# jonH34400/3DBodyAnimation

Measured on AMD Instinct MI355X. Metric: SMPL residual+Jacobian evals/sec (6890v, 10 beta, 24 joints), higher is better.
Workload: dtype f64 residual/Jacobian; f32 mesh (f32 + split-bf16 MFMA blend); 1 GPU; C3: 256 independent frames per GPU, BODY_25 (14 FK joints + 11 vertex landmarks), opt-shape (per-frame beta, 86 cols), GMM prior on, 6890-vertex mesh on; frames_per_gpu=256, keypoints_per_frame=25, n_cols=86

## Files before the change

### 3dbodyanimation_amd/csrc/frame_part_inl.h

```cpp
#pragma once
#include <hip/hip_ext.h>

#include "bodyfit_device.h"
#include "priors_inl.h"

namespace bodyfit {
namespace {

__device__ __forceinline__ void store_through(double* p, double v) {
  __hip_atomic_store(p, v, __ATOMIC_RELAXED, __HIP_MEMORY_SCOPE_SYSTEM);
}
#ifndef BODYFIT_J_THROUGH
#define BODYFIT_J_THROUGH 1
#endif
template <bool kFused>
__device__ __forceinline__ void store_J(double* p, double v, int scope = 0) {
  if constexpr (kFused && !BODYFIT_J_THROUGH) *p = v;
  else if (scope == 1) store_f64_through(p, v);
  else if (scope == 2) *p = v;
  else store_through(p, v);
}


__device__ inline void mul33(const double* A, const double* B, double* C) {
#pragma unroll
  for (int r = 0; r < 3; ++r)
#pragma unroll
    for (int c = 0; c < 3; ++c) C[r * 3 + c] = A[r * 3] * B[c] + A[r * 3 + 1] * B[3 + c] + A[r * 3 + 2] * B[6 + c];
}
__device__ inline void mul33_bt(const double* A, const double* B, double* C) {
#pragma unroll
  for (int r = 0; r < 3; ++r)
#pragma unroll
    for (int c = 0; c < 3; ++c)
      C[r * 3 + c] = A[r * 3] * B[c * 3] + A[r * 3 + 1] * B[c * 3 + 1] + A[r * 3 + 2] * B[c * 3 + 2];
}
__device__ inline void mv3(const double* A, double x0, double x1, double x2, double* y) {
#pragma unroll
  for (int r = 0; r < 3; ++r) y[r] = A[r * 3] * x0 + A[r * 3 + 1] * x1 + A[r * 3 + 2] * x2;
}

__device__ void rodrigues_grad_k(double a0, double a1, double a2, int k, double* R, double* dRk) {
  const double th2 = a0 * a0 + a1 * a1 + a2 * a2;
  if (th2 > 2.220446049250313e-16) {
    const double th = sqrt(th2), ith = 1.0 / th;
    double sh, ch;
    sincos(0.5 * th, &sh, &ch);
    const double st = 2.0 * sh * ch, omc = 2.0 * sh * sh, ct = 1.0 - omc;
    const double w[3] = {a0 * ith, a1 * ith, a2 * ith};
    const double K[9] = {0, -w[2], w[1], w[2], 0, -w[0], -w[1], w[0], 0};
#pragma unroll
    for (int r = 0; r < 3; ++r)
#pragma unroll
      for (int c = 0; c < 3; ++c) R[r * 3 + c] = (r == c ? ct : 0.0) + st * K[r * 3 + c] + omc * w[r] * w[c];
    const double wk = (k == 0) ? w[0] : (k == 1 ? w[1] : w[2]);
    double dw[3];
#pragma unroll
    for (int i = 0; i < 3; ++i) dw[i] = ((i == k ? 1.0 : 0.0) - w[i] * wk) * ith;
    const double dK[9] = {0, -dw[2], dw[1], dw[2], 0, -dw[0], -dw[1], dw[0], 0};
#pragma unroll
    for (int r = 0; r < 3; ++r)
#pragma unroll
      for (int c = 0; c < 3; ++c)
        dRk[r * 3 + c] = (r == c ? -st * wk : 0.0) + ct * wk * K[r * 3 + c] + st * dK[r * 3 + c] +
                         st * wk * w[r] * w[c] + omc * (dw[r] * w[c] + w[r] * dw[c]);
  } else {
    R[0] = 1; R[1] = -a2; R[2] = a1;
    R[3] = a2; R[4] = 1; R[5] = -a0;
    R[6] = -a1; R[7] = a0; R[8] = 1;
#pragma unroll
    for (int i = 0; i < 9; ++i) dRk[i] = 0.0;
    if (k == 0) { dRk[5] = -1; dRk[7] = 1; }
    else if (k == 1) { dRk[2] = 1; dRk[6] = -1; }
    else { dRk[1] = -1; dRk[3] = 1; }
  }
}

__device__ inline double wave_sum(double v) {
#pragma unroll
  for (int off = 32; off > 0; off >>= 1) v += __shfl_down(v, off, 64);
  return v;
}

#ifdef BODYFIT_STAMPS
#define STAMP(i)                                                                              \
  do {                                                                                        \
    if (Pb.dbg && (threadIdx.x & 63) == 0) {                                                  \
      unsigned long long t_;                                                                  \
      asm volatile("s_memtime %0\n\ts_waitcnt lgkmcnt(0)" : "=s"(t_)::"memory");              \
      Pb.dbg[((size_t)f * 8 + (threadIdx.x >> 6)) * 16 + (i)] = t_;                  \
    }                                                                                         \
  } while (0)
#define STAMP_REAL(i)                                                                         \
  do {                                                                                        \
    if (Pb.dbg && (threadIdx.x & 63) == 0) {                                                  \
      unsigned long long t_;                                                                  \
      asm volatile("s_memrealtime %0\n\ts_waitcnt lgkmcnt(0)" : "=s"(t_)::"memory");          \
      Pb.dbg[((size_t)f * 8 + (threadIdx.x >> 6)) * 16 + (i)] = t_;                  \
    }                                                                                         \
  } while (0)
#else
#define STAMP(i)
#define STAMP_REAL(i)
#endif

constexpr int KC = 32;
constexpr int kThreads = 512;

constexpr int OFF_X = 0;
constexpr int OFF_R = OFF_X + 88;
constexpr int OFF_DR = OFF_R + 216;
constexpr int OFF_A = OFF_DR + 648;
constexpr int OFF_P = OFF_A + 216;
constexpr int OFF_O = OFF_P + 72;
constexpr int OFF_JC = OFF_O + 72;
constexpr int OFF_W = OFF_JC + 72;
constexpr int OFF_B = OFF_W + 624;
constexpr int OFF_FEAT = OFF_B + 720;
constexpr int OFF_CAM = OFF_FEAT + 208;
constexpr int OFF_KP = OFF_CAM + 40;
constexpr int OFF_TAB = OFF_KP + KC * 18;
constexpr int OFF_KPUV = OFF_TAB + 64;
constexpr int OFF_DS = OFF_KPUV + 2 * KC;
constexpr int OFF_SC = OFF_DS + 720;
constexpr int OFF_PART = OFF_SC + 720;
constexpr int OFF_T = OFF_PART + 128;
constexpr int OFF_CHAIN = OFF_T + 720;
constexpr int OFF_LM = OFF_CHAIN + 24;
constexpr int LM_VP = 0;
constexpr int LM_Q = 3;
constexpr int LM_A = 6;
constexpr int LM_X = 15;
constexpr int LM_W = 39;
constexpr int LM_J = 47;
constexpr int LM_NW = 51;
constexpr int LM_BETA = 52;
constexpr int LM_PD = 82;
constexpr int LM_STRIDE = 290;
constexpr int TAB_PARENT = 0;
constexpr int TAB_ANC = 24;
constexpr int TAB_KPID = 96;

struct FrameHead {
  const unsigned char* mtab;
  const unsigned char* ptab;
  const double* R0;
  int F, K;
  int dims;
};
static_assert(kMaxJoints < 64 && kMaxShape < 16 && kMaxLandmarks < 64 && 7 + 3 * (kMaxJoints - 1) + kMaxShape < 256,
              "FrameHead::dims: 6 + 4 + 6 + 8 bits for nJ, nS, nL, ncols; beta_stride (0 or nS) in 4");
__host__ __device__ inline int frame_head_dims(int nJ, int nS, int nL, int ncols, int use_shape, int beta_stride, int has_coef) {
  return nJ | (nS << 6) | (nL << 10) | (ncols << 16) | ((use_shape ? 1 : 0) << 24) | (beta_stride << 25) | ((has_coef ? 1 : 0) << 29);
}

struct FusedFrame {
  unsigned* flag;
  unsigned epoch;
  int j_scope;
};

template <bool kFused>
__device__ __forceinline__ void frame_sync() {
  if constexpr (kFused) asm volatile("s_waitcnt lgkmcnt(0)\n\ts_barrier" ::: "memory");
  else __syncthreads();
}

template <bool kFused>
__device__ __forceinline__ void store_operand16(void* p, uint4 v) {
  if constexpr (kFused) {
    typedef __attribute__((ext_vector_type(4))) unsigned int u32x4_;
    const u32x4_ x = {v.x, v.y, v.z, v.w};
    asm volatile("global_store_dwordx4 %0, %1, off sc1\n\ts_nop 1" ::"v"(p), "v"(x) : "memory");
  } else {
    *reinterpret_cast<uint4*>(p) = v;
  }
}

template <bool kFused>
__device__ __forceinline__ void frame_part(const DevModel& M, const DevProblem& Pb, const double* __restrict__ params,
                                           const double* __restrict__ beta, double* __restrict__ r_out,
                                           double* __restrict__ J_out, double* __restrict__ joints_out, const MeshCoef& mc,
                                           int want_jac, double* sm, int f, const FusedFrame& fu, const FrameHead& hd) {
  const int tid = threadIdx.x;
  const int lane = tid & 63, wave = tid >> 6;
  const int nJ = kFused ? (hd.dims & 63) : M.nJ, nS = kFused ? ((hd.dims >> 6) & 15) : M.nS, nL = kFused ? ((hd.dims >> 10) & 63) : M.nL;
  const int ncols = kFused ? ((hd.dims >> 16) & 255) : Pb.ncols;
  const int npose = 7 + 3 * (nJ - 1);
  const bool use_shape = kFused ? (((hd.dims >> 24) & 1) != 0) : (Pb.use_shape != 0);
  const int beta_stride = kFused ? ((hd.dims >> 25) & 15) : Pb.beta_stride;
  const unsigned char* const mtab = kFused ? hd.mtab : M.tabA;
  const unsigned char* const ptab = kFused ? hd.ptab : Pb.ptab;
  const int* const t_parent = reinterpret_cast<const int*>(mtab + kTabParent);
  const unsigned* const t_anc = reinterpret_cast<const unsigned*>(mtab + kTabAnc);
  const unsigned long long* const t_chain = reinterpret_cast<const unsigned long long*>(mtab + kTabChain);
  const int* const t_lm_woff = reinterpret_cast<const int*>(mtab + kTabLmWoff);
  const int* const t_lm_wj = reinterpret_cast<const int*>(mtab + kTabLmWj);
  const double* const t_lm_ww = reinterpret_cast<const double*>(mtab + kTabLmWw);
  const double* const t_lm_vt = reinterpret_cast<const double*>(mtab + kTabLmVt);
  const double* const t_lm_sd = reinterpret_cast<const double*>(mtab + kTabLmSd);
  const double* const t_dS = reinterpret_cast<const double*>(mtab + kTabDS);
  const double* const t_Sc = reinterpret_cast<const double*>(mtab + kTabSc);
  const double* const t_offset = reinterpret_cast<const double*>(mtab + kTabOffset);
  const double* const t_Jc0 = reinterpret_cast<const double*>(mtab + kTabJc0);
  const int t_F = kFused ? hd.F : Pb.F, t_K = kFused ? hd.K : Pb.K;
  const int* const t_kp_offset = reinterpret_cast<const int*>(ptab);
  const int* const t_kp_id = reinterpret_cast<const int*>(ptab + ptab_id_off(t_F));
  const double* const t_kp_uv = reinterpret_cast<const double*>(ptab + ptab_uv_off(t_F, t_K));
  const double* const t_R0 = kFused ? hd.R0 : Pb.R0;
  const int P = M.P;
  double* sx = sm + OFF_X;
  double* sR = sm + OFF_R;
  double* sdR = sm + OFF_DR;
  double* sA = sm + OFF_A;
  double* sP = sm + OFF_P;
  double* sO = sm + OFF_O;
  double* sJc = sm + OFF_JC;
  double* sW = sm + OFF_W;
  double* sB = sm + OFF_B;
  double* sFeat = sm + OFF_FEAT;
  double* sCam = sm + OFF_CAM;
  double* sKp = sm + OFF_KP;
  int* sTab = reinterpret_cast<int*>(sm + OFF_TAB);
  double* sKpUv = sm + OFF_KPUV;
  double* sDS = sm + OFF_DS;
  double* sSc = sm + OFF_SC;
  double* sPart = sm + OFF_PART;
  double* sLm = sm + OFF_LM;
  double* sT = sm + OFF_T;
  double* sLmSd = sLm + nL * LM_STRIDE;
  int* sParent = sTab + TAB_PARENT;
  unsigned* sAnc = reinterpret_cast<unsigned*>(sTab + TAB_ANC);
  int* sKpId = sTab + TAB_KPID;
  unsigned* sKpAnc = reinterpret_cast<unsigned*>(sTab + 48);
  unsigned long long* sChain = reinterpret_cast<unsigned long long*>(sm + OFF_CHAIN);

  STAMP_REAL(10);
  STAMP(0);
#ifdef BODYFIT_STAMPS
  if (Pb.dbg && tid == 0) {
    unsigned xcc;
    asm volatile("s_getreg_b32 %0, hwreg(HW_REG_XCC_ID)" : "=s"(xcc));
    Pb.dbg[((size_t)f * 8) * 16 + 9] = xcc & 0xf;
  }
#endif
  if constexpr (!kFused) {
    if (Pb.frame_flags && !(Pb.frame_flags[f] & Pb.frame_mask)) return;
  }
  constexpr int kLoaders = kThreads;
  constexpr bool loader = true;
  constexpr int kSdPasses = (kMaxLandmarks * 3 * kMaxShape + kThreads - 1) / kThreads;
  constexpr int kPasses = (720 + kLoaders - 1) / kLoaders;
  const bool coef_wave = kFused && wave == 5 && ((hd.dims >> 29) & 1) != 0;
  const int tj_c = min(tid, nJ - 1);
  const int par_in = t_parent[tj_c];
  const unsigned anc_in = t_anc[tj_c];
  const unsigned long long chain_in = t_chain[tj_c];
  const int nlw = nL * kMaxLmNnz, lw_i = min(tid, max(nlw, 1) - 1);
  const double lww_in = t_lm_ww[lw_i];
  const int lwj_in = t_lm_wj[lw_i];
  const int lwo_in = t_lm_woff[lw_i / kMaxLmNnz];
  const int nsd = nL * 3 * nS, nds = nJ * 3 * nS;
  double sd_in[kSdPasses], t0[kPasses], t1[kPasses];
#pragma unroll
  for (int u = 0; u < kSdPasses; ++u) sd_in[u] = t_lm_sd[min(tid + u * kThreads, max(nsd, 1) - 1)];
#pragma unroll
  for (int u = 0; u < kPasses; ++u) {
    const int i = min(tid + u * kLoaders, max(nds, 1) - 1);
    t0[u] = t_dS[i];
    t1[u] = t_Sc[i];
  }
  const int k_begin0 = t_kp_offset[f], nk0 = min(KC, t_kp_offset[f + 1] - k_begin0);
  const int o_i = tid - 128, v_row = tid - 256;
  const bool o_lane = tid >= 128 && o_i < nJ * 3, v_lane = tid >= 256 && v_row < nL * 3;
  double o_pre = 0.0, jc_pre = 0.0, vt_pre = 0.0;
  if (o_lane) { o_pre = t_offset[o_i]; jc_pre = t_Jc0[o_i]; }
  if (v_lane) vt_pre = t_lm_vt[v_row];
  const int cam_lane = tid - 384;
  const bool cam_on = cam_lane >= 0 && cam_lane < 36;
  double r0c0 = 0.0, r0c1 = 0.0, r0c2 = 0.0;
  if (cam_on) {
    const double* R0 = t_R0 + (size_t)f * 9;
    const int c = cam_lane % 3;
    r0c0 = R0[c]; r0c1 = R0[3 + c]; r0c2 = R0[6 + c];
  }
  double x_in = 0.0;
  const bool x_lane = tid >= 128 && tid - 128 < npose, b_lane = tid >= 224 && tid - 224 < nS;
  if (x_lane) x_in = params[(size_t)f * npose + tid - 128];
  if (b_lane) x_in = (use_shape && beta) ? beta[(size_t)f * beta_stride + tid - 224] : 0.0;
  int kp_id0 = 0;
  double kp_u0 = 0.0, kp_v0 = 0.0;
  if (loader) {
    kp_id0 = t_kp_id[k_begin0 + (tid & (KC - 1))];
    kp_u0 = t_kp_uv[2 * (size_t)(k_begin0 + (tid & (KC - 1)))];
    kp_v0 = t_kp_uv[2 * (size_t)(k_begin0 + (tid & (KC - 1))) + 1];
  }
  if (tid < nJ) { sParent[tid] = par_in; sAnc[tid] = anc_in; sChain[tid] = chain_in; }
  volatile int* sWalkDone = reinterpret_cast<volatile int*>(sPart + 104);
  if (tid == 0) *sWalkDone = 0;
  if (tid < nlw) {
    const int l = tid / kMaxLmNnz, i = tid % kMaxLmNnz;
    double* L = sLm + l * LM_STRIDE;
    L[LM_W + i] = lww_in;
    reinterpret_cast<int*>(L + LM_J)[i] = lwj_in;
    if (i == 0) L[LM_NW] = (double)lwo_in;
  }
#pragma unroll
  for (int u = 0; u < kSdPasses; ++u)
    if (tid + u * kThreads < nsd) sLmSd[tid + u * kThreads] = sd_in[u];
#pragma unroll
  for (int u = 0; u < kPasses; ++u) {
    const int i = tid + u * kLoaders;
    if (i < nds) { sDS[i] = t0[u]; sSc[i] = t1[u]; }
  }
  if (x_lane) sx[tid - 128] = x_in;
  if (b_lane) sx[npose + tid - 224] = x_in;
  frame_sync<kFused>();
  if (tid < nk0) {
    sTab[TAB_KPID + tid] = kp_id0;
    sKpUv[2 * tid] = kp_u0;
    sKpUv[2 * tid + 1] = kp_v0;
  }
  const double* sbeta = sx + npose;

  STAMP(1);
  if (tid < 3 * nJ) {
    const int jj = tid / 3, k = tid - 3 * jj;
    const double* aa = (jj == 0) ? (sx + 1) : (sx + 7 + 3 * (jj - 1));
    double R[9], dRk[9];
    rodrigues_grad_k(aa[0], aa[1], aa[2], k, R, dRk);
    if (k == 0) {
#pragma unroll
      for (int i = 0; i < 9; ++i) sR[jj * 9 + i] = R[i];
    }
#pragma unroll
    for (int i = 0; i < 9; ++i) sdR[jj * 27 + k * 9 + i] = dRk[i];
  }
  if (v_lane) {
    const int row = v_row;
    double sv[kMaxShape];
#pragma unroll
    for (int k = 0; k < kMaxShape; ++k) sv[k] = (use_shape && k < nS) ? sLmSd[row * nS + k] : 0.0;
    double acc = vt_pre;
#pragma unroll
    for (int k = 0; k < kMaxShape; ++k) acc += sv[k] * sbeta[min(k, nS > 0 ? nS - 1 : 0)];
    sPart[row] = acc;
  }
  if (coef_wave) {
    float* cf = reinterpret_cast<float*>(sW);
    const int nfeat = 9 * (nJ - 1);
    if (lane < nJ - 1) {
      const float a0 = (float)sx[7 + 3 * lane], a1 = (float)sx[8 + 3 * lane], a2 = (float)sx[9 + 3 * lane];
      const float th2 = a0 * a0 + a1 * a1 + a2 * a2;
      float st = 1.0f, omc = 0.0f, w0 = a0, w1 = a1, w2 = a2;
      if (th2 > 1e-20f) {
        const float ith = rsqrtf(th2), th = th2 * ith;
        float sh, ch;
        sincosf(0.5f * th, &sh, &ch);
        st = 2.0f * sh * ch; omc = 2.0f * sh * sh;
        w0 = a0 * ith; w1 = a1 * ith; w2 = a2 * ith;
      }
      const float on = Pb.pose_blend ? 1.0f : 0.0f;
      float* o = cf + 9 * lane;
      o[0] = on * (omc * (w0 * w0 - 1.0f)); o[1] = on * (omc * w0 * w1 - st * w2); o[2] = on * (omc * w0 * w2 + st * w1);
      o[3] = on * (omc * w1 * w0 + st * w2); o[4] = on * (omc * (w1 * w1 - 1.0f)); o[5] = on * (omc * w1 * w2 - st * w0);
      o[6] = on * (omc * w2 * w0 - st * w1); o[7] = on * (omc * w2 * w1 + st * w0); o[8] = on * (omc * (w2 * w2 - 1.0f));
    } else if (lane >= 32 && lane - 32 < 16 * kBlendKSteps - kPoseFeat) {
      const int i = lane - 32;
      cf[kPoseFeat + i] = (i < nS) ? (float)sbeta[i] : ((i == kMaxShape || i == kMaxShape + 1) ? 1.0f : 0.0f);
    }
    if (lane < 32)
      for (int k = nfeat + lane; k < kPoseFeat; k += 32) cf[k] = 0.0f;
  }
  if (o_lane) {
    const int i = o_i;
    double o = o_pre, jc = jc_pre;
    if (use_shape) {
      for (int k = 0; k < nS; ++k) {
        o += sDS[i * nS + k] * sbeta[k];
        jc += sSc[i * nS + k] * sbeta[k];
      }
    }
    sO[i] = (i < 3) ? 0.0 : o;
    if (i < 3) sPart[100 + i] = o;
    sJc[i] = jc;
  }
  __builtin_amdgcn_s_waitcnt(0x0F70);
  frame_sync<kFused>();

  STAMP(2);
  const int lm_k = lane & 31, lm_l = 2 * wave + (lane >> 5);
  const bool lm_blend = Pb.pose_blend && P > 0;
  auto lm_load = [&](int l, double (&pdv)[27]) {
    const double* row = M.lm_pd + (size_t)min(l, max(nL, 1) - 1) * 27 * 32 + lm_k;
#pragma unroll
    for (int ae = 0; ae < 27; ++ae) pdv[ae] = row[ae * 32];
  };
  auto lm_terms = [&](int l, const double (&pdv)[27]) {
    const int k = min(lm_k + 1, nJ - 1);
    const bool lm_on = l < nL, on = lm_on && lm_k < nJ - 1;
    const double onf = (lm_blend && on) ? 1.0 : 0.0;
    double part[3] = {0.0, 0.0, 0.0};
#pragma unroll
    for (int e = 0; e < 9; ++e) {
      const double fe = (sR[k * 9 + e] - ((e % 4 == 0) ? 1.0 : 0.0)) * onf;
#pragma unroll
      for (int a = 0; a < 3; ++a) part[a] += pdv[a * 9 + e] * fe;
    }
    if (want_jac) {
#pragma unroll
      for (int c = 0; c < 3; ++c) {
        const double* d = sdR + k * 27 + c * 9;
        double h[3] = {0.0, 0.0, 0.0};
#pragma unroll
        for (int e = 0; e < 9; ++e) {
          const double de = d[e] * onf;
#pragma unroll
          for (int a = 0; a < 3; ++a) h[a] += pdv[a * 9 + e] * de;
        }
        if (on) {
          double* o = sLm + l * LM_STRIDE + LM_PD + (3 * (k - 1) + c) * 3;
          o[0] = h[0]; o[1] = h[1]; o[2] = h[2];
        }
      }
    }
#pragma unroll
    for (int a = 0; a < 3; ++a) {
#pragma unroll
      for (int off = 16; off > 0; off >>= 1) part[a] += __shfl_xor(part[a], off, 32);
    }
    if (lm_on && lm_k == 0) {
#pragma unroll
      for (int a = 0; a < 3; ++a) sLm[l * LM_STRIDE + LM_VP + a] = sPart[l * 3 + a] + part[a];
    }
  };
  const bool lm_wave0 = 2 * wave < nL, lm_wave1 = 2 * wave + 16 < nL;
  if (tid < 9) sA[tid] = (tid % 4 == 0) ? 1.0 : 0.0;
  if (tid >= 16 && tid < 19) sP[tid - 16] = 0.0;
  if (tid >= 32 && tid - 32 < 3 * nS) { sB[tid - 32] = 0.0; sT[tid - 32] = 0.0; }
  if (wave == 0) {
    asm volatile("s_waitcnt lgkmcnt(0)" ::: "memory");
    if (lane == 0) __hip_atomic_fetch_add(const_cast<int*>(sWalkDone), 1, __ATOMIC_RELAXED, __HIP_MEMORY_SCOPE_WORKGROUP);
  }
  if (coef_wave) {
    const float* cf = reinterpret_cast<const float*>(sW);
    if (lane < kBlendKSteps * 4) {
      const int kstep = lane >> 2, h = (lane >> 1) & 1, hl = lane & 1;
      const float4 v0 = *reinterpret_cast<const float4*>(cf + 16 * kstep + 8 * h);
      const float4 v1 = *reinterpret_cast<const float4*>(cf + 16 * kstep + 8 * h + 4);
      const float x[8] = {v0.x, v0.y, v0.z, v0.w, v1.x, v1.y, v1.z, v1.w};
      uint32_t pk[4];
#pragma unroll
      for (int q = 0; q < 4; ++q) {
        uint16_t b[2];
#pragma unroll
        for (int t = 0; t < 2; ++t) {
          const uint16_t hi = f32_to_bf16(x[2 * q + t]);
          b[t] = hl == 0 ? hi : f32_to_bf16(x[2 * q + t] - bf16_to_f32(hi));
        }
        pk[q] = (uint32_t)b[0] | ((uint32_t)b[1] << 16);
      }
      const int ftile = f / kFTile, phi = f % kFTile;
      const int row = 8 * (phi >> 3) + 4 * (phi & 1) + ((phi >> 1) & 3);
      uint4* dst = reinterpret_cast<uint4*>(reinterpret_cast<unsigned char*>(mc.featA) + ((size_t)ftile * kBlendKSteps + kstep) * 2048 +
                                            feat_frag_off(h * 32 + row, hl));
      store_operand16<true>(dst, make_uint4(pk[0], pk[1], pk[2], pk[3]));
    }
    asm volatile("s_waitcnt vmcnt(0)" ::: "memory");
    STAMP_REAL(14);
    if (lane == 0)
      (void)__hip_atomic_fetch_add(fu.flag + (size_t)(f / kFTile) * kUnitCounterStride + kUnitCoefOffset, 1u, __ATOMIC_RELAXED,
                                   __HIP_MEMORY_SCOPE_AGENT);
  }
  double pdv0[27];
  if (lm_wave0) lm_load(lm_l, pdv0);
  for (int i = tid; i < 208; i += kThreads) {
    double v = 0.0;
    if (i < 9 * (nJ - 1)) v = sR[9 + i] - (((i % 9) % 4 == 0) ? 1.0 : 0.0);
    sFeat[i] = v;
  }
  auto walk = [&](int kind, int j, int sel, bool on) {
    j = on ? j : 1;
    const double* tab = (kind == 2) ? sDS : sO;
    const int stride = (kind == 2) ? nS : 1, off = (kind == 2) ? sel : 0;
    const double m = (kind == 0) ? 0.0 : 1.0;
    const double* ini = (kind == 0) ? (sR + j * 9 + sel) : (tab + (j * 3) * stride + off);
    const int istride = (kind == 0) ? 3 : stride;
    double v0 = ini[0], v1 = ini[istride], v2 = ini[2 * istride];
    unsigned long long ch = on ? sChain[j] : 0ull;
    int k = (int)(ch & 31ull);
    double Rc[9], oc[3];
    auto fetch = [&](int kk, double (&Rn)[9], double (&on_)[3]) {
#pragma unroll
      for (int e = 0; e < 9; ++e) Rn[e] = sR[kk * 9 + e];
#pragma unroll
      for (int a3 = 0; a3 < 3; ++a3) on_[a3] = tab[(kk * 3 + a3) * stride + off];
    };
    fetch(k, Rc, oc);
    while (k > 0) {
      ch >>= 5;
      const int kn = (int)(ch & 31ull);
      double Rn[9], on_[3];
      fetch(kn, Rn, on_);
      const double t0 = Rc[0] * v0 + Rc[1] * v1 + Rc[2] * v2 + m * oc[0];
      const double t1 = Rc[3] * v0 + Rc[4] * v1 + Rc[5] * v2 + m * oc[1];
      const double t2 = Rc[6] * v0 + Rc[7] * v1 + Rc[8] * v2 + m * oc[2];
      v0 = t0; v1 = t1; v2 = t2;
#pragma unroll
      for (int e = 0; e < 9; ++e) Rc[e] = Rn[e];
      oc[0] = on_[0]; oc[1] = on_[1]; oc[2] = on_[2];
      k = kn;
    }
    if (!on) return;
    if (kind == 0) { sA[j * 9 + sel] = v0; sA[j * 9 + 3 + sel] = v1; sA[j * 9 + 6 + sel] = v2; }
    else if (kind == 1) { sP[j * 3] = v0; sP[j * 3 + 1] = v1; sP[j * 3 + 2] = v2; }
    else {
      sB[(j * 3 + 0) * nS + sel] = v0; sB[(j * 3 + 1) * nS + sel] = v1; sB[(j * 3 + 2) * nS + sel] = v2;
      double c[3];
      mv3(sA + j * 9, sSc[(j * 3 + 0) * nS + sel], sSc[(j * 3 + 1) * nS + sel], sSc[(j * 3 + 2) * nS + sel], c);
      sT[(j * 3 + 0) * nS + sel] = v0 - c[0]; sT[(j * 3 + 1) * nS + sel] = v1 - c[1]; sT[(j * 3 + 2) * nS + sel] = v2 - c[2];
    }
  };
  if (!kFused && wave == 0 && mc.featA) {
    const int ftile = f / kFTile, phi = f % kFTile;
    const int row = Pb.feat_perm ? (8 * (phi >> 3) + 4 * (phi & 1) + ((phi >> 1) & 3)) : phi;
    if (lane >= 8 && lane - 8 < kBlendKSteps * 4) {
      const int wl = lane - 8;
      const int kstep = wl >> 2, h = (wl >> 1) & 1, hl = wl & 1;
      const int k0 = kstep * 16 + 8 * h;
      const int nfeat = 9 * (nJ - 1);
      double vr[8], vb[8];
#pragma unroll
      for (int u = 0; u < 8; ++u) {
        vr[u] = sR[9 + min(k0 + u, nfeat - 1)];
        vb[u] = sbeta[min(max(k0 + u - kPoseFeat, 0), max(nS, 1) - 1)];
      }
      uint32_t pk[4];
#pragma unroll
      for (int jj = 0; jj < 4; ++jj) {
        uint16_t b[2];
#pragma unroll
        for (int u = 0; u < 2; ++u) {
          const int k = k0 + 2 * jj + u;
          const float xr = (Pb.pose_blend && k < nfeat) ? (float)(vr[2 * jj + u] - (((k % 9) % 4 == 0) ? 1.0 : 0.0)) : 0.0f;
          const float xb = (k - kPoseFeat < nS) ? (float)vb[2 * jj + u]
                                                : ((k == kPoseFeat + kMaxShape || k == kPoseFeat + kMaxShape + 1) ? 1.0f : 0.0f);
          const float x = (k < kPoseFeat) ? xr : xb;
          const uint16_t hi = f32_to_bf16(x);
          b[u] = hl == 0 ? hi : f32_to_bf16(x - bf16_to_f32(hi));
        }
        pk[jj] = (uint32_t)b[0] | ((uint32_t)b[1] << 16);
      }
      uint4* dst = reinterpret_cast<uint4*>(reinterpret_cast<unsigned char*>(mc.featA) + ((size_t)ftile * kBlendKSteps + kstep) * 2048 +
                                            feat_frag_off(h * 32 + row, hl));
      store_operand16<kFused>(dst, make_uint4(pk[0], pk[1], pk[2], pk[3]));
    }
  }
  if (cam_on) {
    const int mtx = cam_lane / 9, e = cam_lane % 9, r = e / 3;
    const double* Lm = (mtx == 0) ? sR : (sdR + (mtx - 1) * 9);
    sCam[cam_lane] = Lm[r * 3] * r0c0 + Lm[r * 3 + 1] * r0c1 + Lm[r * 3 + 2] * r0c2;
  }
  {
    const int nA = 3 * (nJ - 1), nP = nJ - 1;
    const int nA6 = (nA + 1) / 2, nP6 = (nP + 1) / 2;
    if (wave == 6 || wave == 7) {
      const int a0 = wave == 6 ? 0 : nA6, na = wave == 6 ? nA6 : nA - nA6;
      const int p0 = wave == 6 ? 0 : nP6, np = wave == 6 ? nP6 : nP - nP6;
      const bool isA = lane < na, isP = !isA && lane - na < np;
      const int item = isA ? a0 + lane : p0 + (lane - na);
      walk(isA ? 0 : 1, isA ? 1 + item / 3 : 1 + item, isA ? item % 3 : 0, isA || isP);
    }
  }
  if (wave == 6) {
    asm volatile("s_waitcnt lgkmcnt(0)" ::: "memory");
    if (lane == 0) __hip_atomic_fetch_add(const_cast<int*>(sWalkDone), 256, __ATOMIC_RELAXED, __HIP_MEMORY_SCOPE_WORKGROUP);
  }
  if (wave == 7) {
    STAMP(13);
    for (int spin = 0; spin < (1 << 20) && *sWalkDone < 257; ++spin) __builtin_amdgcn_s_sleep(1);
    asm volatile("" ::: "memory");
    STAMP(14);
    const double s_ = sx[0];
    const double* Rr0_ = sCam;
    for (int it = lane; it < 3 * nJ; it += 64) {
      const int jj = it / 3, r = it - 3 * jj;
      const double* Aj = sA + jj * 9;
      const double a0 = Rr0_[r * 3], a1 = Rr0_[r * 3 + 1], a2 = Rr0_[r * 3 + 2];
      double q[3];
      mv3(Aj, sJc[jj * 3], sJc[jj * 3 + 1], sJc[jj * 3 + 2], q);
      const double p0 = sP[jj * 3], p1 = sP[jj * 3 + 1], p2 = sP[jj * 3 + 2];
      if (mc.skinT) {
        const double ra0 = a0 * Aj[0] + a1 * Aj[3] + a2 * Aj[6];
        const double ra1 = a0 * Aj[1] + a1 * Aj[4] + a2 * Aj[7];
        const double ra2 = a0 * Aj[2] + a1 * Aj[5] + a2 * Aj[8];
        const double tr = a0 * (p0 - q[0]) + a1 * (p1 - q[1]) + a2 * (p2 - q[2]);
        float4* T = reinterpret_cast<float4*>(mc.skinT + (size_t)f * nJ * 12) + it;
        store_operand16<kFused>(T, make_uint4(__float_as_uint((float)(s_ * ra0)), __float_as_uint((float)(s_ * ra1)),
                                              __float_as_uint((float)(s_ * ra2)), __float_as_uint((float)(s_ * tr + sx[4 + r]))));
      }
      if (joints_out) joints_out[(size_t)f * nJ * 3 + it] = s_ * (a0 * p0 + a1 * p1 + a2 * p2) + sx[4 + r];
    }
    STAMP(15);
    if constexpr (kFused) {
      asm volatile("s_waitcnt vmcnt(0)" ::: "memory");
      STAMP_REAL(9);
      if (lane == 0)
        (void)__hip_atomic_fetch_add(fu.flag + (size_t)(f / kFTile) * kUnitCounterStride, 1u, __ATOMIC_RELAXED, __HIP_MEMORY_SCOPE_AGENT);
      STAMP_REAL(12);
    }
  }
  if (lm_wave0) lm_terms(lm_l, pdv0);
  if (lm_wave1) {
    double pdv1[27];
    lm_load(lm_l + 16, pdv1);
    lm_terms(lm_l + 16, pdv1);
  }
  STAMP(3);
  frame_sync<kFused>();

  STAMP(4);
  if (use_shape && want_jac) {
    for (int it = tid - 192; it >= 0 && tid < 448 && it < nS * (nJ - 1); it += 256) walk(2, 1 + it / nS, it % nS, true);
  }
  if (want_jac && tid < 3 * (nJ - 1)) {
    const int k = 1 + tid / 3, c = tid % 3, p = sParent[k];
    double T1[9], T2[9], Wm[9];
    mul33_bt(sdR + k * 27 + c * 9, sR + k * 9, T1);
    mul33(sA + p * 9, T1, T2);
    mul33_bt(T2, sA + p * 9, Wm);
#pragma unroll
    for (int e = 0; e < 9; ++e) sW[tid * 9 + e] = Wm[e];
  }
  if (wave == 2 && lane < nL) {
    double* L = sLm + lane * LM_STRIDE;
    const int* Lj = reinterpret_cast<const int*>(L + LM_J);
    double q[3] = {0, 0, 0}, Ab[9] = {0, 0, 0, 0, 0, 0, 0, 0, 0};
    const int nw = (int)L[LM_NW];
    for (int i = 0; i < nw; ++i) {
      const int j = Lj[i];
      const double w = L[LM_W + i];
      double xj[3];
      mv3(sA + j * 9, L[LM_VP] - sJc[j * 3], L[LM_VP + 1] - sJc[j * 3 + 1], L[LM_VP + 2] - sJc[j * 3 + 2], xj);
#pragma unroll
      for (int a = 0; a < 3; ++a) {
        xj[a] += sP[j * 3 + a];
        q[a] += w * xj[a];
        L[LM_X + i * 3 + a] = xj[a];
      }
#pragma unroll
      for (int e = 0; e < 9; ++e) Ab[e] += w * sA[j * 9 + e];
    }
#pragma unroll
    for (int a = 0; a < 3; ++a) L[LM_Q + a] = q[a];
#pragma unroll
    for (int e = 0; e < 9; ++e) L[LM_A + e] = Ab[e];
  }
  if (wave == 2 && M.lm_gcount) {
    const int cnt = (lane < nL) ? M.lm_gcount[lane] : 0;
    if (cnt > 1) {
      double* L = sLm + lane * LM_STRIDE;
      double q0 = L[LM_Q], q1 = L[LM_Q + 1], q2 = L[LM_Q + 2];
      for (int i = 1; i < cnt; ++i) {
        const double* Li = L + i * LM_STRIDE;
        q0 += Li[LM_Q]; q1 += Li[LM_Q + 1]; q2 += Li[LM_Q + 2];
      }
      L[LM_Q] = q0; L[LM_Q + 1] = q1; L[LM_Q + 2] = q2;
    }
  }
  frame_sync<kFused>();
  const double s = sx[0];
  const double* Rr0 = sCam;
  const double* dRr0 = sCam + 9;

  const int k_begin = k_begin0, k_end = k_begin0 + (Pb.kp_offset[f + 1] - k_begin0);
  const bool fold = Pb.beta_partials != nullptr && want_jac && ncols > npose && nS == kMaxShape;
  auto stage_kp = [&](int tid, int kc0) {
    {
      const int kg = kc0 + tid;
      const bool first = kc0 == k_begin;
      const int id = first ? sKpId[tid] : Pb.kp_id[kg];
      const double u_obs = first ? sKpUv[2 * tid] : Pb.kp_uv[2 * (size_t)kg];
      const double v_obs = first ? sKpUv[2 * tid + 1] : Pb.kp_uv[2 * (size_t)kg + 1];
      sKpId[tid] = id;
      sKpAnc[tid] = (id < nJ) ? sAnc[id] : 0u;
      double q[3];
      if (id < nJ) {
        if (id == 0 || sParent[id] < 0) {
#pragma unroll
          for (int a = 0; a < 3; ++a) q[a] = sPart[100 + a];
        } else {
#pragma unroll
          for (int a = 0; a < 3; ++a) q[a] = sP[id * 3 + a];
        }
      } else {
#pragma unroll
        for (int a = 0; a < 3; ++a) q[a] = sLm[(id - nJ) * LM_STRIDE + LM_Q + a];
      }
      double z[3];
      mv3(Rr0, q[0], q[1], q[2], z);
      const double X0 = s * z[0] + sx[4], X1 = s * z[1] + sx[5], X2 = s * z[2] + sx[6];
      const double iz = 1.0 / X2;
      const double res0 = Pb.fx * X0 * iz + Pb.cx - u_obs, res1 = Pb.fy * X1 * iz + Pb.cy - v_obs;
      r_out[2 * (size_t)kg] = res0;
      r_out[2 * (size_t)kg + 1] = res1;
      if (fold) {
        const double sq = res0 * res0 + res1 * res1, d2 = Pb.huber * Pb.huber;
        const bool outl = Pb.huber > 0.0 && sq > d2;
        const double rt = sqrt(sq);
        sKpUv[2 * tid] = res0;
        sKpUv[2 * tid + 1] = res1;
        sFeat[tid] = outl ? sqrt(Pb.huber / rt) : 1.0;
        sFeat[KC + tid] = 0.5 * (outl ? 2.0 * Pb.huber * rt - d2 : sq);
      }
      double* kp = sKp + tid * 18;
      const double dpi[6] = {Pb.fx * iz, 0.0, -Pb.fx * X0 * iz * iz, 0.0, Pb.fy * iz, -Pb.fy * X1 * iz * iz};
#pragma unroll
      for (int a = 0; a < 3; ++a) { kp[a] = q[a]; kp[3 + a] = z[a]; }
#pragma unroll
      for (int i = 0; i < 6; ++i) kp[6 + i] = dpi[i];
#pragma unroll
      for (int rr = 0; rr < 2; ++rr)
#pragma unroll
        for (int c = 0; c < 3; ++c)
          kp[12 + rr * 3 + c] = s * (dpi[rr * 3] * Rr0[c] + dpi[rr * 3 + 1] * Rr0[3 + c] + dpi[rr * 3 + 2] * Rr0[6 + c]);
    }
  };
  STAMP(5);
  if (wave == 6 && lane < min(KC, k_end - k_begin)) stage_kp(lane, k_begin);
  if (nL > 0 && want_jac) {
    for (int l = lm_l; l < nL; l += 16) {
      if (lm_k < nJ - 1) {
        const int k = lm_k + 1;
        const double* L = sLm + l * LM_STRIDE;
        const double* Ab = L + LM_A;
        const int* Lj = reinterpret_cast<const int*>(L + LM_J);
        const int nw = (int)L[LM_NW];
        const double pk0 = sP[k * 3], pk1 = sP[k * 3 + 1], pk2 = sP[k * 3 + 2];
        double a0 = 0, a1 = 0, a2 = 0;
        for (int i = 0; i < nw; ++i) {
          const int j = Lj[i];
          if (j == k || ((sAnc[j] >> k) & 1u)) {
            const double w = L[LM_W + i];
            a0 += w * (L[LM_X + i * 3] - pk0);
            a1 += w * (L[LM_X + i * 3 + 1] - pk1);
            a2 += w * (L[LM_X + i * 3 + 2] - pk2);
          }
        }
#pragma unroll
        for (int c = 0; c < 3; ++c) {
          double* o = sLm + l * LM_STRIDE + LM_PD + (3 * lm_k + c) * 3;
          const double* Wm = sW + (3 * lm_k + c) * 9;
          double t[3];
          mv3(Ab, o[0], o[1], o[2], t);
          o[0] = t[0] + Wm[0] * a0 + Wm[1] * a1 + Wm[2] * a2;
          o[1] = t[1] + Wm[3] * a0 + Wm[4] * a1 + Wm[5] * a2;
          o[2] = t[2] + Wm[6] * a0 + Wm[7] * a1 + Wm[8] * a2;
        }
      }
    }
    if (use_shape) {
      for (int it = kThreads - 1 - tid; it < nL * nS; it += kThreads) {
        const int l = it / nS, k = it % nS;
        const double* L = sLm + l * LM_STRIDE;
        const int* Lj = reinterpret_cast<const int*>(L + LM_J);
        double d[3];
        mv3(L + LM_A, sLmSd[(l * 3 + 0) * nS + k], sLmSd[(l * 3 + 1) * nS + k], sLmSd[(l * 3 + 2) * nS + k], d);
#pragma unroll
        for (int i = 0; i < kMaxLmNnz; ++i) {
          const int j = Lj[i];
          const double w = L[LM_W + i];
          d[0] += w * sT[(j * 3 + 0) * nS + k]; d[1] += w * sT[(j * 3 + 1) * nS + k]; d[2] += w * sT[(j * 3 + 2) * nS + k];
        }
        double* o = sLm + l * LM_STRIDE + LM_BETA + k * 3;
        o[0] = d[0]; o[1] = d[1]; o[2] = d[2];
      }
    }
  }

  STAMP(6);
  if (M.lm_gcount && want_jac && nL > 0) {
    frame_sync<kFused>();
    constexpr int kWords = LM_PD + 207 - LM_BETA;
    static_assert(LM_PD == LM_BETA + 30, "LM_BETA and LM_PD are adjacent");
    for (int it = tid; it < nL * kWords; it += kThreads) {
      const int l = it / kWords, w = it - l * kWords;
      const int cnt = M.lm_gcount[l];
      if (cnt > 1) {
        double* o = sLm + l * LM_STRIDE + LM_BETA + w;
        double v = o[0];
        for (int i = 1; i < cnt; ++i) v += o[i * LM_STRIDE];
        o[0] = v;
      }
    }
  }
  double* sJb = sdR;
  double fold_acc = 0.0;
  typedef __attribute__((ext_vector_type(4))) double fold_d4;
  fold_d4 fold_gram = {0.0, 0.0, 0.0, 0.0};
  for (int kc0 = k_begin; kc0 < k_end; kc0 += KC) {
    const int nk = min(KC, k_end - kc0);
    frame_sync<kFused>();
    if (kc0 != k_begin) {
      if (tid < nk) stage_kp(tid, kc0);
      frame_sync<kFused>();
    }
    STAMP(7);
    if (want_jac) {
      const int njc = npose - 7;
      const int ngrp = kThreads / njc;
      if (tid < ngrp * njc) {
        const int g = tid / njc, kc = tid - g * njc, k = 1 + kc / 3;
        double Wm[9];
#pragma unroll
        for (int e9 = 0; e9 < 9; ++e9) Wm[e9] = sW[kc * 9 + e9];
        const double pk0 = sP[k * 3], pk1 = sP[k * 3 + 1], pk2 = sP[k * 3 + 2];
        for (int kk = g; kk < nk; kk += ngrp) {
          const int kg = kc0 + kk;
          const int id = sKpId[kk];
          const unsigned am = sKpAnc[kk];
          const double* kp = sKp + kk * 18;
          const double* G = kp + 12;
          double d0 = 0.0, d1 = 0.0, d2 = 0.0;
          if (id < nJ) {
            if ((am >> k) & 1u) {
              const double x0 = kp[0] - pk0, x1 = kp[1] - pk1, x2 = kp[2] - pk2;
              d0 = Wm[0] * x0 + Wm[1] * x1 + Wm[2] * x2;
              d1 = Wm[3] * x0 + Wm[4] * x1 + Wm[5] * x2;
              d2 = Wm[6] * x0 + Wm[7] * x1 + Wm[8] * x2;
            }
          } else {
            const double* o = sLm + (id - nJ) * LM_STRIDE + LM_PD + kc * 3;
            d0 = o[0]; d1 = o[1]; d2 = o[2];
          }
          store_J<kFused>(J_out + (size_t)(2 * kg) * ncols + 7 + kc, G[0] * d0 + G[1] * d1 + G[2] * d2, fu.j_scope);
          store_J<kFused>(J_out + (size_t)(2 * kg + 1) * ncols + 7 + kc, G[3] * d0 + G[4] * d1 + G[5] * d2, fu.j_scope);
        }
      }
      const int nsc = 7 + (ncols - npose);
      for (int e = tid; e < nk * nsc; e += kThreads) {
        const int kk = e / nsc, c = e - kk * nsc;
        const int kg = kc0 + kk;
        const int id = sKpId[kk];
        const double* kp = sKp + kk * 18;
        const double* G = kp + 12;
        double j0, j1;
        int col;
        if (c == 0) {
          col = 0;
          j0 = kp[6] * kp[3] + kp[7] * kp[4] + kp[8] * kp[5];
          j1 = kp[9] * kp[3] + kp[10] * kp[4] + kp[11] * kp[5];
        } else if (c < 4) {
          col = c;
          double t[3];
          mv3(dRr0 + (c - 1) * 9, kp[0], kp[1], kp[2], t);
          j0 = s * (kp[6] * t[0] + kp[7] * t[1] + kp[8] * t[2]);
          j1 = s * (kp[9] * t[0] + kp[10] * t[1] + kp[11] * t[2]);
        } else if (c < 7) {
          col = c;
          j0 = kp[6 + (c - 4)];
          j1 = kp[9 + (c - 4)];
        } else {
          const int k = c - 7;
          col = npose + k;
          double d0 = 0.0, d1 = 0.0, d2 = 0.0;
          if (use_shape) {
            if (id < nJ) {
              if (id == 0 || sParent[id] < 0) {
                d0 = sDS[(id * 3 + 0) * nS + k]; d1 = sDS[(id * 3 + 1) * nS + k]; d2 = sDS[(id * 3 + 2) * nS + k];
              } else {
                d0 = sB[(id * 3 + 0) * nS + k]; d1 = sB[(id * 3 + 1) * nS + k]; d2 = sB[(id * 3 + 2) * nS + k];
              }
            } else {
              const double* o = sLm + (id - nJ) * LM_STRIDE + LM_BETA + k * 3;
              d0 = o[0]; d1 = o[1]; d2 = o[2];
            }
          }
          j0 = G[0] * d0 + G[1] * d1 + G[2] * d2;
          j1 = G[3] * d0 + G[4] * d1 + G[5] * d2;
        }
        store_J<kFused>(J_out + (size_t)(2 * kg) * ncols + col, j0, fu.j_scope);
        store_J<kFused>(J_out + (size_t)(2 * kg + 1) * ncols + col, j1, fu.j_scope);
        if (fold && c >= 7) { sJb[(2 * kk) * kMaxShape + c - 7] = j0; sJb[(2 * kk + 1) * kMaxShape + c - 7] = j1; }
      }
    }
    if (fold) {
      frame_sync<kFused>();
      if (wave == 0) {
        const int col = lane & 15, kq = lane >> 4;
        for (int s0 = 0; s0 < (2 * nk + 3) / 4; s0 += 4) {
          double vv[4];
#pragma unroll
          for (int u = 0; u < 4; ++u) {
            const int row = 4 * (s0 + u) + kq;
            const bool on = row < 2 * nk;
            const double sw = on ? sFeat[row >> 1] : 0.0;
            const double x = (on && col < nS) ? sJb[row * kMaxShape + col] : ((on && col == 10) ? sKpUv[row] : 0.0);
            vv[u] = sw * x;
          }
#pragma unroll
          for (int u = 0; u < 4; ++u) fold_gram = __builtin_amdgcn_mfma_f64_16x16x4f64(vv[u], vv[u], fold_gram, 0, 0, 0);
        }
      } else if (tid == 64) {
        for (int kk = 0; kk < nk; ++kk) fold_acc += sFeat[KC + kk];
      }
    }
  }
  if (fold) {
    double* out = Pb.beta_partials + (size_t)f * kReducePartial;
    if (wave == 0) {
#pragma unroll
      for (int q = 0; q < 4; ++q) {
        const int gi = (lane >> 4) + 4 * q, gj = lane & 15;
        if (gi < 10 && gj >= gi && gj <= 10) {
          double* o = out + fold_slot_gram(gi, gj);
          if constexpr (kFused) store_f64_through(o, fold_gram[q]); else *o = fold_gram[q];
        }
      }
    } else if (tid == 64) {
      if constexpr (kFused) store_f64_through(out + fold_slot_cost(0), fold_acc); else out[fold_slot_cost(0)] = fold_acc;
    }
  }
  STAMP(8);
  STAMP_REAL(11);
}

constexpr size_t frame_lds_bytes(int nL) { return (size_t)(OFF_LM + nL * (LM_STRIDE + 3 * kMaxShape)) * sizeof(double); }

}
}
```

Baseline: 12.23 million evals/s.

## Split sim3/shape Jacobian loop by column class and use float reciprocal division

Splits the single mixed-branch loop over keypoint Jacobian columns into three loops: rotation columns, scale/translation columns and shape columns. Each starts at a different thread offset, which removes divergent branching within waves. Integer divisions by small runtime counts are replaced with a float-reciprocal approximation, and the landmark pose-blend derivative skips its multiply-accumulate when blending is off. Off-by-default CENSUS assembly markers are also added for static instruction counting. The float division trick relies on small operands staying exact.

```diff
diff --git a/3dbodyanimation_amd/csrc/frame_part_inl.h b/3dbodyanimation_amd/csrc/frame_part_inl.h
--- a/3dbodyanimation_amd/csrc/frame_part_inl.h
+++ b/3dbodyanimation_amd/csrc/frame_part_inl.h
@@ -76,12 +76,21 @@
   }
 }
 
+__device__ __forceinline__ int small_div(int x, int n) {
+  return (int)(((float)x + 0.5f) * __builtin_amdgcn_rcpf((float)n));
+}
+
 __device__ inline double wave_sum(double v) {
 #pragma unroll
   for (int off = 32; off > 0; off >>= 1) v += __shfl_down(v, off, 64);
   return v;
 }
 
+#ifdef BODYFIT_CENSUS
+#define CENSUS(tag) asm volatile("; CENSUS " tag)
+#else
+#define CENSUS(tag)
+#endif
 #ifdef BODYFIT_STAMPS
 #define STAMP(i)                                                                              \
   do {                                                                                        \
@@ -100,7 +109,11 @@
     }                                                                                         \
   } while (0)
 #else
+#ifdef BODYFIT_CENSUS
+#define STAMP(i) CENSUS("stamp_" #i)
+#else
 #define STAMP(i)
+#endif
 #define STAMP_REAL(i)
 #endif
 
@@ -325,6 +338,7 @@
 
   STAMP(1);
   if (tid < 3 * nJ) {
+    CENSUS("B.rodrigues");
     const int jj = tid / 3, k = tid - 3 * jj;
     const double* aa = (jj == 0) ? (sx + 1) : (sx + 7 + 3 * (jj - 1));
     double R[9], dRk[9];
@@ -336,7 +350,9 @@
 #pragma unroll
     for (int i = 0; i < 9; ++i) sdR[jj * 27 + k * 9 + i] = dRk[i];
   }
+  CENSUS("B.common");
   if (v_lane) {
+    CENSUS("B.lm_rest");
     const int row = v_row;
     double sv[kMaxShape];
 #pragma unroll
@@ -346,7 +362,9 @@
     for (int k = 0; k < kMaxShape; ++k) acc += sv[k] * sbeta[min(k, nS > 0 ? nS - 1 : 0)];
     sPart[row] = acc;
   }
+  CENSUS("B.common");
   if (coef_wave) {
+    CENSUS("B.coef");
     float* cf = reinterpret_cast<float*>(sW);
     const int nfeat = 9 * (nJ - 1);
     if (lane < nJ - 1) {
@@ -372,19 +390,24 @@
     if (lane < 32)
       for (int k = nfeat + lane; k < kPoseFeat; k += 32) cf[k] = 0.0f;
   }
+  CENSUS("B.common");
   if (o_lane) {
+    CENSUS("B.offsets");
     const int i = o_i;
     double o = o_pre, jc = jc_pre;
     if (use_shape) {
       for (int k = 0; k < nS; ++k) {
+        CENSUS("B.offsets_loop");
         o += sDS[i * nS + k] * sbeta[k];
         jc += sSc[i * nS + k] * sbeta[k];
       }
+      CENSUS("B.offsets");
     }
     sO[i] = (i < 3) ? 0.0 : o;
     if (i < 3) sPart[100 + i] = o;
     sJc[i] = jc;
   }
+  CENSUS("B.common");
   __builtin_amdgcn_s_waitcnt(0x0F70);
   frame_sync<kFused>();
 
@@ -412,11 +435,13 @@
       for (int c = 0; c < 3; ++c) {
         const double* d = sdR + k * 27 + c * 9;
         double h[3] = {0.0, 0.0, 0.0};
-#pragma unroll
-        for (int e = 0; e < 9; ++e) {
-          const double de = d[e] * onf;
-#pragma unroll
-          for (int a = 0; a < 3; ++a) h[a] += pdv[a * 9 + e] * de;
+        if (lm_blend) {
+#pragma unroll
+          for (int e = 0; e < 9; ++e) {
+            const double de = d[e];
+#pragma unroll
+            for (int a = 0; a < 3; ++a) h[a] += pdv[a * 9 + e] * de;
+          }
         }
         if (on) {
           double* o = sLm + l * LM_STRIDE + LM_PD + (3 * (k - 1) + c) * 3;
@@ -443,6 +468,7 @@
     if (lane == 0) __hip_atomic_fetch_add(const_cast<int*>(sWalkDone), 1, __ATOMIC_RELAXED, __HIP_MEMORY_SCOPE_WORKGROUP);
   }
   if (coef_wave) {
+    CENSUS("C.coef_publish");
     const float* cf = reinterpret_cast<const float*>(sW);
     if (lane < kBlendKSteps * 4) {
       const int kstep = lane >> 2, h = (lane >> 1) & 1, hl = lane & 1;
@@ -472,13 +498,17 @@
       (void)__hip_atomic_fetch_add(fu.flag + (size_t)(f / kFTile) * kUnitCounterStride + kUnitCoefOffset, 1u, __ATOMIC_RELAXED,
                                    __HIP_MEMORY_SCOPE_AGENT);
   }
+  CENSUS("C.common");
   double pdv0[27];
-  if (lm_wave0) lm_load(lm_l, pdv0);
+  if (lm_wave0) { CENSUS("C.lm_load"); lm_load(lm_l, pdv0); }
+  CENSUS("C.common");
   for (int i = tid; i < 208; i += kThreads) {
+    CENSUS("C.feat");
     double v = 0.0;
     if (i < 9 * (nJ - 1)) v = sR[9 + i] - (((i % 9) % 4 == 0) ? 1.0 : 0.0);
     sFeat[i] = v;
   }
+  CENSUS("C.common");
   auto walk = [&](int kind, int j, int sel, bool on) {
     j = on ? j : 1;
     const double* tab = (kind == 2) ? sDS : sO;
@@ -498,6 +528,7 @@
     };
     fetch(k, Rc, oc);
     while (k > 0) {
+      CENSUS("walk_level");
       ch >>= 5;
       const int kn = (int)(ch & 31ull);
       double Rn[9], on_[3];
@@ -511,6 +542,7 @@
       oc[0] = on_[0]; oc[1] = on_[1]; oc[2] = on_[2];
       k = kn;
     }
+    CENSUS("walk_tail");
     if (!on) return;
     if (kind == 0) { sA[j * 9 + sel] = v0; sA[j * 9 + 3 + sel] = v1; sA[j * 9 + 6 + sel] = v2; }
     else if (kind == 1) { sP[j * 3] = v0; sP[j * 3 + 1] = v1; sP[j * 3 + 2] = v2; }
@@ -522,6 +554,7 @@
     }
   };
   if (!kFused && wave == 0 && mc.featA) {
+    CENSUS("C.coef_two_launch");
     const int ftile = f / kFTile, phi = f % kFTile;
     const int row = Pb.feat_perm ? (8 * (phi >> 3) + 4 * (phi & 1) + ((phi >> 1) & 3)) : phi;
     if (lane >= 8 && lane - 8 < kBlendKSteps * 4) {
@@ -556,7 +589,9 @@
       store_operand16<kFused>(dst, make_uint4(pk[0], pk[1], pk[2], pk[3]));
     }
   }
+  CENSUS("C.common");
   if (cam_on) {
+    CENSUS("C.cam");
     const int mtx = cam_lane / 9, e = cam_lane % 9, r = e / 3;
     const double* Lm = (mtx == 0) ? sR : (sdR + (mtx - 1) * 9);
     sCam[cam_lane] = Lm[r * 3] * r0c0 + Lm[r * 3 + 1] * r0c1 + Lm[r * 3 + 2] * r0c2;
@@ -564,7 +599,9 @@
   {
     const int nA = 3 * (nJ - 1), nP = nJ - 1;
     const int nA6 = (nA + 1) / 2, nP6 = (nP + 1) / 2;
+    CENSUS("C.common");
     if (wave == 6 || wave == 7) {
+      CENSUS("C.walk");
       const int a0 = wave == 6 ? 0 : nA6, na = wave == 6 ? nA6 : nA - nA6;
       const int p0 = wave == 6 ? 0 : nP6, np = wave == 6 ? nP6 : nP - nP6;
       const bool isA = lane < na, isP = !isA && lane - na < np;
@@ -572,11 +609,13 @@
       walk(isA ? 0 : 1, isA ? 1 + item / 3 : 1 + item, isA ? item % 3 : 0, isA || isP);
     }
   }
+  CENSUS("C.common");
   if (wave == 6) {
     asm volatile("s_waitcnt lgkmcnt(0)" ::: "memory");
     if (lane == 0) __hip_atomic_fetch_add(const_cast<int*>(sWalkDone), 256, __ATOMIC_RELAXED, __HIP_MEMORY_SCOPE_WORKGROUP);
   }
   if (wave == 7) {
+    CENSUS("C.transforms");
     STAMP(13);
     for (int spin = 0; spin < (1 << 20) && *sWalkDone < 257; ++spin) __builtin_amdgcn_s_sleep(1);
     asm volatile("" ::: "memory");
@@ -584,6 +623,7 @@
     const double s_ = sx[0];
     const double* Rr0_ = sCam;
     for (int it = lane; it < 3 * nJ; it += 64) {
+      CENSUS("C.transforms_loop");
       const int jj = it / 3, r = it - 3 * jj;
       const double* Aj = sA + jj * 9;
       const double a0 = Rr0_[r * 3], a1 = Rr0_[r * 3 + 1], a2 = Rr0_[r * 3 + 2];
@@ -601,6 +641,7 @@
       }
       if (joints_out) joints_out[(size_t)f * nJ * 3 + it] = s_ * (a0 * p0 + a1 * p1 + a2 * p2) + sx[4 + r];
     }
+    CENSUS("C.transforms");
     STAMP(15);
     if constexpr (kFused) {
       asm volatile("s_waitcnt vmcnt(0)" ::: "memory");
@@ -610,20 +651,30 @@
       STAMP_REAL(12);
     }
   }
-  if (lm_wave0) lm_terms(lm_l, pdv0);
+  CENSUS("C.common");
+  if (lm_wave0) { CENSUS("C.lm_terms"); lm_terms(lm_l, pdv0); }
+  CENSUS("C.common");
   if (lm_wave1) {
+    CENSUS("C.lm_second");
     double pdv1[27];
     lm_load(lm_l + 16, pdv1);
     lm_terms(lm_l + 16, pdv1);
   }
+  CENSUS("C.common");
   STAMP(3);
   frame_sync<kFused>();
 
   STAMP(4);
   if (use_shape && want_jac) {
-    for (int it = tid - 192; it >= 0 && tid < 448 && it < nS * (nJ - 1); it += 256) walk(2, 1 + it / nS, it % nS, true);
-  }
+    for (int it = tid - 192; it >= 0 && tid < 448 && it < nS * (nJ - 1); it += 256) {
+      CENSUS("D.walkB");
+      const int jb = small_div(it, nS);
+      walk(2, 1 + jb, it - jb * nS, true);
+    }
+  }
+  CENSUS("D.common");
   if (want_jac && tid < 3 * (nJ - 1)) {
+    CENSUS("D.W");
     const int k = 1 + tid / 3, c = tid % 3, p = sParent[k];
     double T1[9], T2[9], Wm[9];
     mul33_bt(sdR + k * 27 + c * 9, sR + k * 9, T1);
@@ -632,12 +683,15 @@
 #pragma unroll
     for (int e = 0; e < 9; ++e) sW[tid * 9 + e] = Wm[e];
   }
+  CENSUS("D.common");
   if (wave == 2 && lane < nL) {
+    CENSUS("D.lm_lbs");
     double* L = sLm + lane * LM_STRIDE;
     const int* Lj = reinterpret_cast<const int*>(L + LM_J);
     double q[3] = {0, 0, 0}, Ab[9] = {0, 0, 0, 0, 0, 0, 0, 0, 0};
     const int nw = (int)L[LM_NW];
     for (int i = 0; i < nw; ++i) {
+      CENSUS("D.lm_lbs_loop");
       const int j = Lj[i];
       const double w = L[LM_W + i];
       double xj[3];
@@ -651,12 +705,15 @@
 #pragma unroll
       for (int e = 0; e < 9; ++e) Ab[e] += w * sA[j * 9 + e];
     }
+    CENSUS("D.lm_lbs");
 #pragma unroll
     for (int a = 0; a < 3; ++a) L[LM_Q + a] = q[a];
 #pragma unroll
     for (int e = 0; e < 9; ++e) L[LM_A + e] = Ab[e];
   }
+  CENSUS("D.common");
   if (wave == 2 && M.lm_gcount) {
+    CENSUS("D.lm_rows");
     const int cnt = (lane < nL) ? M.lm_gcount[lane] : 0;
     if (cnt > 1) {
       double* L = sLm + lane * LM_STRIDE;
@@ -668,6 +725,7 @@
       L[LM_Q] = q0; L[LM_Q + 1] = q1; L[LM_Q + 2] = q2;
     }
   }
+  CENSUS("D.common");
   frame_sync<kFused>();
   const double s = sx[0];
   const double* Rr0 = sCam;
@@ -727,9 +785,11 @@
     }
   };
   STAMP(5);
-  if (wave == 6 && lane < min(KC, k_end - k_begin)) stage_kp(lane, k_begin);
+  if (wave == 6 && lane < min(KC, k_end - k_begin)) { CENSUS("E.stage_kp"); stage_kp(lane, k_begin); }
+  CENSUS("E.common");
   if (nL > 0 && want_jac) {
     for (int l = lm_l; l < nL; l += 16) {
+      CENSUS("E.lm_theta");
       if (lm_k < nJ - 1) {
         const int k = lm_k + 1;
         const double* L = sLm + l * LM_STRIDE;
@@ -739,6 +799,7 @@
         const double pk0 = sP[k * 3], pk1 = sP[k * 3 + 1], pk2 = sP[k * 3 + 2];
         double a0 = 0, a1 = 0, a2 = 0;
         for (int i = 0; i < nw; ++i) {
+          CENSUS("E.lm_theta_loop");
           const int j = Lj[i];
           if (j == k || ((sAnc[j] >> k) & 1u)) {
             const double w = L[LM_W + i];
@@ -747,6 +808,7 @@
             a2 += w * (L[LM_X + i * 3 + 2] - pk2);
           }
         }
+        CENSUS("E.lm_theta");
 #pragma unroll
         for (int c = 0; c < 3; ++c) {
           double* o = sLm + l * LM_STRIDE + LM_PD + (3 * lm_k + c) * 3;
@@ -759,9 +821,11 @@
         }
       }
     }
+    CENSUS("E.common");
     if (use_shape) {
       for (int it = kThreads - 1 - tid; it < nL * nS; it += kThreads) {
-        const int l = it / nS, k = it % nS;
+        CENSUS("E.lm_beta");
+        const int l = small_div(it, nS), k = it - l * nS;
         const double* L = sLm + l * LM_STRIDE;
         const int* Lj = reinterpret_cast<const int*>(L + LM_J);
         double d[3];
@@ -775,6 +839,7 @@
         double* o = sLm + l * LM_STRIDE + LM_BETA + k * 3;
         o[0] = d[0]; o[1] = d[1]; o[2] = d[2];
       }
+      CENSUS("E.common");
     }
   }
 
@@ -784,6 +849,7 @@
     constexpr int kWords = LM_PD + 207 - LM_BETA;
     static_assert(LM_PD == LM_BETA + 30, "LM_BETA and LM_PD are adjacent");
     for (int it = tid; it < nL * kWords; it += kThreads) {
+      CENSUS("E.lm_rows_merge");
       const int l = it / kWords, w = it - l * kWords;
       const int cnt = M.lm_gcount[l];
       if (cnt > 1) {
@@ -793,6 +859,7 @@
         o[0] = v;
       }
     }
+    CENSUS("E.common");
   }
   double* sJb = sdR;
   double fold_acc = 0.0;
@@ -802,20 +869,24 @@
     const int nk = min(KC, k_end - kc0);
     frame_sync<kFused>();
     if (kc0 != k_begin) {
+      CENSUS("F.stage_next");
       if (tid < nk) stage_kp(tid, kc0);
       frame_sync<kFused>();
     }
+    CENSUS("F.common");
     STAMP(7);
     if (want_jac) {
       const int njc = npose - 7;
-      const int ngrp = kThreads / njc;
+      const int ngrp = small_div(kThreads, njc);
       if (tid < ngrp * njc) {
-        const int g = tid / njc, kc = tid - g * njc, k = 1 + kc / 3;
+        CENSUS("F.joint_setup");
+        const int g = small_div(tid, njc), kc = tid - g * njc, k = 1 + kc / 3;
         double Wm[9];
 #pragma unroll
         for (int e9 = 0; e9 < 9; ++e9) Wm[e9] = sW[kc * 9 + e9];
         const double pk0 = sP[k * 3], pk1 = sP[k * 3 + 1], pk2 = sP[k * 3 + 2];
         for (int kk = g; kk < nk; kk += ngrp) {
+          CENSUS("F.joint_loop");
           const int kg = kc0 + kk;
           const int id = sKpId[kk];
           const unsigned am = sKpAnc[kk];
@@ -837,56 +908,63 @@
           store_J<kFused>(J_out + (size_t)(2 * kg + 1) * ncols + 7 + kc, G[3] * d0 + G[4] * d1 + G[5] * d2, fu.j_scope);
         }
       }
-      const int nsc = 7 + (ncols - npose);
-      for (int e = tid; e < nk * nsc; e += kThreads) {
-        const int kk = e / nsc, c = e - kk * nsc;
+      CENSUS("F.common");
+      for (int e = tid; e < nk * 3; e += kThreads) {
+        CENSUS("F.sim3_rot");
+        const int kk = e / 3, c = e - 3 * kk;
+        const int kg = kc0 + kk;
+        const double* kp = sKp + kk * 18;
+        double t[3];
+        mv3(dRr0 + c * 9, kp[0], kp[1], kp[2], t);
+        store_J<kFused>(J_out + (size_t)(2 * kg) * ncols + 1 + c, s * (kp[6] * t[0] + kp[7] * t[1] + kp[8] * t[2]), fu.j_scope);
+        store_J<kFused>(J_out + (size_t)(2 * kg + 1) * ncols + 1 + c, s * (kp[9] * t[0] + kp[10] * t[1] + kp[11] * t[2]), fu.j_scope);
+      }
+      CENSUS("F.common");
+      for (int e = tid - 128; e >= 0 && e < nk * 4; e += kThreads) {
+        CENSUS("F.sim3_scale_trans");
+        const int kk = e >> 2, q = e & 3;
+        const int kg = kc0 + kk;
+        const double* kp = sKp + kk * 18;
+        const double d0 = kp[6 + max(q - 1, 0)], d1 = kp[9 + max(q - 1, 0)];
+        const double j0 = (q == 0) ? kp[6] * kp[3] + kp[7] * kp[4] + kp[8] * kp[5] : d0;
+        const double j1 = (q == 0) ? kp[9] * kp[3] + kp[10] * kp[4] + kp[11] * kp[5] : d1;
+        const int col = (q == 0) ? 0 : 3 + q;
+        store_J<kFused>(J_out + (size_t)(2 * kg) * ncols + col, j0, fu.j_scope);
+        store_J<kFused>(J_out + (size_t)(2 * kg + 1) * ncols + col, j1, fu.j_scope);
+      }
+      CENSUS("F.common");
+      const int nshape = ncols - npose;
+      for (int e = kThreads - 1 - tid; e < nk * nshape; e += kThreads) {
+        CENSUS("F.shape");
+        const int kk = small_div(e, nshape), k = e - kk * nshape;
         const int kg = kc0 + kk;
         const int id = sKpId[kk];
-        const double* kp = sKp + kk * 18;
-        const double* G = kp + 12;
-        double j0, j1;
-        int col;
-        if (c == 0) {
-          col = 0;
-          j0 = kp[6] * kp[3] + kp[7] * kp[4] + kp[8] * kp[5];
-          j1 = kp[9] * kp[3] + kp[10] * kp[4] + kp[11] * kp[5];
-        } else if (c < 4) {
-          col = c;
-          double t[3];
-          mv3(dRr0 + (c - 1) * 9, kp[0], kp[1], kp[2], t);
-          j0 = s * (kp[6] * t[0] + kp[7] * t[1] + kp[8] * t[2]);
-          j1 = s * (kp[9] * t[0] + kp[10] * t[1] + kp[11] * t[2]);
-        } else if (c < 7) {
-          col = c;
-          j0 = kp[6 + (c - 4)];
-          j1 = kp[9 + (c - 4)];
-        } else {
-          const int k = c - 7;
-          col = npose + k;
-          double d0 = 0.0, d1 = 0.0, d2 = 0.0;
-          if (use_shape) {
-            if (id < nJ) {
-              if (id == 0 || sParent[id] < 0) {
-                d0 = sDS[(id * 3 + 0) * nS + k]; d1 = sDS[(id * 3 + 1) * nS + k]; d2 = sDS[(id * 3 + 2) * nS + k];
-              } else {
-                d0 = sB[(id * 3 + 0) * nS + k]; d1 = sB[(id * 3 + 1) * nS + k]; d2 = sB[(id * 3 + 2) * nS + k];
-              }
+        const double* G = sKp + kk * 18 + 12;
+        double d0 = 0.0, d1 = 0.0, d2 = 0.0;
+        if (use_shape) {
+          if (id < nJ) {
+            if (id == 0 || sParent[id] < 0) {
+              d0 = sDS[(id * 3 + 0) * nS + k]; d1 = sDS[(id * 3 + 1) * nS + k]; d2 = sDS[(id * 3 + 2) * nS + k];
             } else {
-              const double* o = sLm + (id - nJ) * LM_STRIDE + LM_BETA + k * 3;
-              d0 = o[0]; d1 = o[1]; d2 = o[2];
+              d0 = sB[(id * 3 + 0) * nS + k]; d1 = sB[(id * 3 + 1) * nS + k]; d2 = sB[(id * 3 + 2) * nS + k];
             }
+          } else {
+            const double* o = sLm + (id - nJ) * LM_STRIDE + LM_BETA + k * 3;
+            d0 = o[0]; d1 = o[1]; d2 = o[2];
           }
-          j0 = G[0] * d0 + G[1] * d1 + G[2] * d2;
-          j1 = G[3] * d0 + G[4] * d1 + G[5] * d2;
-        }
-        store_J<kFused>(J_out + (size_t)(2 * kg) * ncols + col, j0, fu.j_scope);
-        store_J<kFused>(J_out + (size_t)(2 * kg + 1) * ncols + col, j1, fu.j_scope);
-        if (fold && c >= 7) { sJb[(2 * kk) * kMaxShape + c - 7] = j0; sJb[(2 * kk + 1) * kMaxShape + c - 7] = j1; }
-      }
+        }
+        const double j0 = G[0] * d0 + G[1] * d1 + G[2] * d2;
+        const double j1 = G[3] * d0 + G[4] * d1 + G[5] * d2;
+        store_J<kFused>(J_out + (size_t)(2 * kg) * ncols + npose + k, j0, fu.j_scope);
+        store_J<kFused>(J_out + (size_t)(2 * kg + 1) * ncols + npose + k, j1, fu.j_scope);
+        if (fold) { sJb[(2 * kk) * kMaxShape + k] = j0; sJb[(2 * kk + 1) * kMaxShape + k] = j1; }
+      }
+      CENSUS("F.common");
     }
     if (fold) {
       frame_sync<kFused>();
       if (wave == 0) {
+        CENSUS("F.fold_gram");
         const int col = lane & 15, kq = lane >> 4;
         for (int s0 = 0; s0 < (2 * nk + 3) / 4; s0 += 4) {
           double vv[4];
@@ -902,8 +980,10 @@
           for (int u = 0; u < 4; ++u) fold_gram = __builtin_amdgcn_mfma_f64_16x16x4f64(vv[u], vv[u], fold_gram, 0, 0, 0);
         }
       } else if (tid == 64) {
+        CENSUS("F.fold_cost");
         for (int kk = 0; kk < nk; ++kk) fold_acc += sFeat[KC + kk];
       }
+      CENSUS("F.common");
     }
   }
   if (fold) {
```

After: 12.22 million evals/s, median of 2. No clear change (-0.0%).
